# siyi-wind/MDViT

Hardware: AMD Instinct MI355X
Metric: 512x512 images/sec MDViT train step (fwd+bwd, two-sweep, AdamW) (higher is better)
Workload: dtype bf16x3 (fp32 storage; GEMM operands split hi+lo bf16, fp32 accumulate); 1 GPU; MDViT Sup+MLPFM train step, 4 domain(s) x bs=4 per GPU, 512x512, drop_rate=0.1 drop_path=0.1, bf16x3 GEMMs, data-parallel x1

## Files before the change

### include/mdvit_hip.h

```cpp
#ifndef MDVIT_HIP_H
#define MDVIT_HIP_H

#include <stddef.h>
#include <stdint.h>

#ifdef __cplusplus
extern "C" {
#endif

#define MDVIT_ABI_VERSION 1

enum {
    MDVIT_OK = 0,
    MDVIT_E_SHAPE = 1,
    MDVIT_E_DTYPE = 2,
    MDVIT_E_ALIGN = 3,
    MDVIT_E_WORKSPACE = 4,
    MDVIT_E_HIP = 5
};

enum { MDVIT_EPI_NONE = 0, MDVIT_EPI_GELU_DUAL = 1, MDVIT_EPI_DGELU = 2 };
enum { MDVIT_ACT_NONE = 0, MDVIT_ACT_HSWISH = 1, MDVIT_ACT_RELU = 2 };

const char* mdvit_last_error(void);
// ... 274 lines not shown
    float* dW1[MDVIT_DA_MANY_MAX]; float* db1[MDVIT_DA_MANY_MAX]; float* dW2[MDVIT_DA_MANY_MAX]; float* db2[MDVIT_DA_MANY_MAX];
} MdvitDaManyGrads;
size_t mdvit_da_many_ws_bytes(const MdvitDaMany* m, int32_t B);
int mdvit_da_bwd_many(const MdvitDaMany* m, const MdvitDaManyGrads* g, const float* label, float scale, void* ws, size_t ws_bytes, int32_t B, int32_t D, void* stream);
size_t mdvit_da_ws_bytes(int32_t B, int32_t hid, int32_t C);
int mdvit_da_bwd(const float* label, const float* W1, const float* b1, const float* W2, const float* b2, const float* a,
                 const float* e, float scale, float* dW1, float* db1, float* dW2, float* db2, void* ws, size_t ws_bytes,
                 int32_t B, int32_t D, int32_t hid, int32_t C, int32_t heads, void* stream);

size_t mdvit_factoratt_ws_bytes(int32_t B, int32_t N, int32_t C, int32_t heads);
int mdvit_factoratt_fwd(const float* qkv, const float* w3, const float* b3, const float* w5, const float* b5,
                        const float* w7, const float* b7, const float* a, float* out, float* U, float* kmax, float* ksum, float* Mmat,
                        void* ws, size_t ws_bytes, int32_t B, int32_t H, int32_t W, int32_t C, int32_t heads,
                        int32_t s3, int32_t s5, int32_t s7, void* stream);
int mdvit_factoratt_bwd(const float* dout, const float* qkv, const float* out, const float* U,
                        const float* w3, const float* b3, const float* w5, const float* b5, const float* w7, const float* b7,
                        const float* a, const float* kmax, const float* ksum, const float* Mmat,
                        float* dqkv, float* e, float* dw3, float* db3, float* dw5, float* db5, float* dw7, float* db7,
                        void* ws, size_t ws_bytes, int32_t B, int32_t H, int32_t W, int32_t C, int32_t heads,
                        int32_t s3, int32_t s5, int32_t s7, void* stream);
int mdvit_factoratt_wgrad(const float* qkv, void* ws, size_t ws_bytes, float* dw3, float* db3, float* dw5, float* db5,
                          float* dw7, float* db7, int32_t B, int32_t H, int32_t W, int32_t C, int32_t heads,
                          int32_t s3, int32_t s5, int32_t s7, int32_t accumulate, void* stream);

int mdvit_seg_losses_fwd(const float* out, const float* aux, const float* label, double* sums, float* losses, int64_t n, void* stream);
int mdvit_seg_losses_sums(const float* out, const float* aux, const float* label, double* sums, int64_t n, void* stream);
int mdvit_seg_losses_final(const double* sums, float* losses, int64_t n_total, int32_t has_aux, void* stream);
int mdvit_seg_losses_bwd(const float* out, const float* aux, const float* label, const double* sums, const float* g,
                         float* dout, float* daux, int64_t n, float dice_gain, void* stream);
int mdvit_seg_losses_bwd3(const float* out, const float* aux, const float* label, const double* sums, const float* g0, const float* g1, const float* g2,
                          float* dout, float* daux, int64_t n, float dice_gain, void* stream);
int mdvit_seg_losses_groups_sums(const float* out, const float* aux, const float* label, double* sums, int64_t n, int32_t G, void* stream);
int mdvit_seg_losses_groups_final(const double* sums, float* losses, float* per_group, int64_t n_total, int32_t has_aux, int32_t G, void* stream);
int mdvit_seg_losses_groups_bwd(const float* out, const float* aux, const float* label, const double* sums, const float* g0, const float* g1, const float* g2,
                                float* dout, float* daux, int64_t n, int32_t G, float dice_gain, void* stream);

int mdvit_seg_metrics(const float* out, const float* aux, const float* label, uint64_t* counts, float* metrics, int64_t n, void* stream);
size_t mdvit_eval_ws_bytes(int32_t G);
int mdvit_eval_accumulate(const float* out, const float* aux, const float* label, const int32_t* images, const int32_t* domains, int32_t G,
                          int64_t n_per_image, int32_t num_domains, double* acc, int64_t* counts, float* batch_rows, void* ws, size_t ws_bytes, void* stream);
int mdvit_eval_table(const double* acc, int32_t num_domains, float* table, void* stream);
size_t mdvit_eval_images_ws_bytes(int32_t n, int64_t HW);
int mdvit_eval_images(const float* out, const float* aux, const float* label, int32_t n, int64_t HW, int64_t* counts, uint64_t* bits, uint64_t* aux_bits,
                      void* ws, size_t ws_bytes, void* stream);
size_t mdvit_eval_structure_ws_bytes(int32_t n, int32_t H, int32_t W);
int mdvit_eval_structure(const float* pred, const float* label, int32_t n, int32_t H, int32_t W, double* loss, double* sums, void* ws, size_t ws_bytes,
// ... 102 lines not shown
```

### mdvit_amd/_lib.py

```python
from __future__ import annotations

import ctypes as C
import os
import re
from typing import List

_HERE = os.path.dirname(os.path.abspath(__file__))
LIB_PATH = os.environ.get("MDVIT_HIP_LIB") or os.path.join(_HERE, "lib", "libmdvit_hip.so")
HEADER_PATH = os.path.join(_HERE, "..", "include", "mdvit_hip.h")

EPI_NONE, EPI_GELU_DUAL, EPI_DGELU = 0, 1, 2
ACT_NONE, ACT_HSWISH, ACT_RELU = 0, 1, 2

f32p = C.c_void_p
vp = C.c_void_p
i32 = C.c_int32
i64 = C.c_int64
u32 = C.c_uint32
f32 = C.c_float


class GemmDesc(C.Structure):
    _fields_ = [
        ("A", vp), ("B", vp), ("C", vp), ("C2", vp),
# ... 187 lines not shown
    "mdvit_gconv2_3x3_fwd": [vp, vp, vp, vp, i32, i32, i32, i32, vp],
    "mdvit_gconv2_3x3_bwd": [vp, vp, vp, vp, vp, vp, vp, vp, C.c_size_t, i32, i32, i32, i32, i32, vp],
    "mdvit_im2col3x3": [vp, vp, i32, i32, i32, i32, i32, i32, vp],
    "mdvit_col2im3x3": [vp, vp, i32, i32, i32, i32, i32, i32, vp],
    "mdvit_dropout_f32": [vp, vp, i64, f32, u32, u32, vp, vp],
    "mdvit_stemconv_fwd": [vp, vp, vp, i32, i32, i32, i32, i32, vp],
    "mdvit_stemconv_wgrad": [vp, vp, vp, vp, C.c_size_t, i32, i32, i32, i32, i32, i32, vp],
    "mdvit_bn_rowdot_fwd": [vp, vp, vp, vp, vp, vp, vp, vp, i32, i32, i32, f32, u32, u32, vp, i32, vp],
    "mdvit_bn_rowdot_bwd": [vp, vp, vp, vp, vp, vp, vp, vp, vp, vp, vp, vp, vp, C.c_size_t, i32, i32, i32, i32, f32, u32, u32, vp, i32, vp],
    "mdvit_bn_stats": [vp, vp, C.c_size_t, vp, vp, vp, vp, vp, i32, i32, i32, i32, f32, f32, vp],
    "mdvit_bn_eval_prep": [vp, vp, vp, vp, i32, f32, vp],
    "mdvit_bn_apply": [vp, vp, vp, vp, vp, vp, i32, i32, i32, i32, i32, f32, u32, u32, vp, i32, vp],
    "mdvit_bn_bwd": [vp, vp, vp, vp, vp, vp, vp, vp, vp, vp, C.c_size_t, i32, i32, i32, i32, i32, i32, f32, u32, u32, vp, i32, vp],
    "mdvit_upsample_multi_fwd": [vp, vp, vp, i32, vp, vp, i32, i32, i32, i32, vp],
    "mdvit_upsample_multi_bwd": [vp, vp, vp, vp, i32, vp, C.c_size_t, i32, i32, i32, i32, vp],
    "mdvit_upsample_fwd": [vp, vp, vp, i32, i32, i32, i32, i32, i32, vp],
    "mdvit_upsample_bwd": [vp, vp, vp, C.c_size_t, i32, i32, i32, i32, i32, i32, vp],
    "mdvit_upsample_bwd_config": [i32],
    "mdvit_da_fwd": [vp, vp, vp, vp, vp, vp, i32, i32, i32, i32, i32, vp],
    "mdvit_da_bwd": [vp] * 7 + [f32] + [vp] * 4 + [vp, C.c_size_t] + [i32] * 5 + [vp],
    "mdvit_factoratt_fwd": [vp] * 13 + [vp, C.c_size_t] + [i32] * 8 + [vp],
    "mdvit_factoratt_wgrad": [vp, vp, C.c_size_t] + [vp] * 6 + [i32] * 9 + [vp],
    "mdvit_factoratt_bwd": [vp] * 22 + [vp, C.c_size_t] + [i32] * 8 + [vp],
    "mdvit_seg_losses_fwd": [vp, vp, vp, vp, vp, i64, vp],
    "mdvit_adamw_step": [vp, i32, i32, vp, vp, f32, f32, f32, f32, i32, vp],
    "mdvit_adam_step": [vp, i32, i32, vp, vp, f32, f32, f32, f32, i32, i32, vp],
    "mdvit_table_pack": [vp, i32, vp, i32, vp],
    "mdvit_table_unpack": [vp, i32, vp, i32, vp],
    "mdvit_seg_metrics": [vp, vp, vp, vp, vp, i64, vp],
    "mdvit_eval_accumulate": [vp, vp, vp, C.POINTER(i32), C.POINTER(i32), i32, i64, i32, vp, vp, vp, vp, C.c_size_t, vp],
    "mdvit_eval_table": [vp, i32, vp, vp],
    "mdvit_eval_images": [vp, vp, vp, i32, i64, vp, vp, vp, vp, C.c_size_t, vp],
    "mdvit_eval_structure": [vp, vp, i32, i32, i32, vp, vp, vp, C.c_size_t, vp],
    "mdvit_image_normalize_u8": [vp, vp, i32, i32, i32, vp],
    "mdvit_augment_normalize_u8": [vp, vp, vp, vp, vp, vp, i32, i32, i32, vp],
    "mdvit_augment_probe_taps": [f32, f32, i32, i32, C.POINTER(i32), C.POINTER(f32)],
    "mdvit_gather_resize_u8": [vp, vp, vp, vp, i32, vp, i32, vp, vp, i64, i32, i32, i32, i32, i32, vp],
    "mdvit_seg_losses_sums": [vp, vp, vp, vp, i64, vp],
    "mdvit_seg_losses_final": [vp, vp, i64, i32, vp],
    "mdvit_seg_losses_bwd": [vp, vp, vp, vp, vp, vp, vp, i64, f32, vp],
    "mdvit_seg_losses_bwd3": [vp, vp, vp, vp, vp, vp, vp, vp, vp, i64, f32, vp],
    "mdvit_seg_losses_groups_sums": [vp, vp, vp, vp, i64, i32, vp],
    "mdvit_seg_losses_groups_final": [vp, vp, vp, i64, i32, i32, vp],
    "mdvit_seg_losses_groups_bwd": [vp, vp, vp, vp, vp, vp, vp, vp, vp, i64, i32, f32, vp],
    "mdvit_se_adapter_fwd": [C.POINTER(SeAdapterDesc), vp, vp, vp, vp, C.c_size_t, vp],
    "mdvit_se_adapter_bwd": [C.POINTER(SeAdapterDesc)] + [vp] * 10 + [vp, C.c_size_t, vp],
# ... 39 lines not shown
        return _lib
    if not os.path.exists(LIB_PATH):
        raise MdvitHipError(
            f"{LIB_PATH} is missing: build it with `python -m mdvit_amd.build` (hipcc, gfx950). "
            "mdvit_amd has no CPU or PyTorch fallback.")
    lib = C.CDLL(LIB_PATH)
    try:
        _attach_prototypes(lib)
    except AttributeError as e:
        raise MdvitHipError(f"{LIB_PATH} is stale ({e}): rebuild it with `python -m mdvit_amd.build`.") from None
    _lib = lib
    while _on_load:
        _on_load.pop(0)(lib)
    return lib


def _attach_prototypes(lib):
    lib.mdvit_last_error.restype = C.c_char_p
    lib.mdvit_last_error.argtypes = []
    lib.mdvit_version.restype = C.c_int
    lib.mdvit_version.argtypes = []
    lib.mdvit_factoratt_ws_bytes.restype = C.c_size_t
    lib.mdvit_factoratt_ws_bytes.argtypes = [i32, i32, i32, i32]
    lib.mdvit_gemm_ws_bytes.restype = C.c_size_t
    lib.mdvit_gemm_ws_bytes.argtypes = [C.POINTER(GemmDesc)]
    lib.mdvit_gate_bwd_ws_bytes.restype = C.c_size_t
    lib.mdvit_gate_bwd_ws_bytes.argtypes = [i32, i64, i32, i32]
    lib.mdvit_gemm_planes_ws_bytes.restype = C.c_size_t
    lib.mdvit_gemm_planes_ws_bytes.argtypes = [C.POINTER(PlaneGemmDesc)]
    lib.mdvit_bn_rowdot_ws_bytes.restype = C.c_size_t
    lib.mdvit_bn_rowdot_ws_bytes.argtypes = [i32, i32]
    lib.mdvit_bn_ws_bytes.restype = C.c_size_t
    lib.mdvit_bn_ws_bytes.argtypes = [i32, i32, i32]
    lib.mdvit_upsample_multi_bwd_ws_bytes.restype = C.c_size_t
    lib.mdvit_upsample_multi_bwd_ws_bytes.argtypes = [vp, i32, i32, i32, i32]
    lib.mdvit_upsample_bwd_ws_bytes.restype = C.c_size_t
    lib.mdvit_upsample_bwd_ws_bytes.argtypes = [i32] * 6
    lib.mdvit_partials_ws_bytes.restype = C.c_size_t
    lib.mdvit_partials_ws_bytes.argtypes = [i32]
    lib.mdvit_mlp_rc_wgrad_ws_bytes.restype = C.c_size_t
    lib.mdvit_mlp_rc_wgrad_ws_bytes.argtypes = [i32, i32, i32]
    lib.mdvit_block_save_bytes.restype = C.c_size_t
    lib.mdvit_block_save_bytes.argtypes = [C.POINTER(BlockDesc)]
    lib.mdvit_block_fwd_ws_bytes.restype = C.c_size_t
    lib.mdvit_block_fwd_ws_bytes.argtypes = [C.POINTER(BlockDesc)]
    lib.mdvit_block_bwd_ws_bytes.restype = C.c_size_t
# ... 39 lines not shown
```

### mdvit_amd/csrc/attn.hip

```cpp
#include "common.h"
#include "conv_tile.h"

namespace {

constexpr int FA_T = 64;

struct FaGeom {
    int B, H, W, N, C, heads, Ch, s3, s5, s7;
    float scale;
};

typedef float fap_f32x16 __attribute__((ext_vector_type(16)));

template <int CH, bool SOFTMAX>
__global__ __launch_bounds__(256) void fa_partial_kernel(const float* __restrict__ X, long ldx, const float* __restrict__ Y, long ldy,
                                                         const float* __restrict__ ysc, float yscale,
                                                         float* __restrict__ ws_m, float* __restrict__ ws_s, float* __restrict__ ws_P,
                                                         FaGeom g, int NT, int NSUB,
                                                         const float* __restrict__ outp = nullptr, float* __restrict__ dU = nullptr, float* __restrict__ e_part = nullptr) {
    constexpr int GW = CH < 32 ? 32 : CH, NB = (GW + 31) / 32, GQ = GW / 4;
    constexpr int STAGE = 2 * FA_T * GW, RED = 4 * NB * 32 * NB * 32;
    __shared__ __attribute__((aligned(16))) float sm[(STAGE > RED ? STAGE : RED) + 3 * NB * 32 + (SOFTMAX ? 2 * 256 : 0)];
    float* xs = sm;
    float* ys = sm + FA_T * GW;
// ... 1066 lines not shown
}

extern "C" int mdvit_factoratt_wgrad(const float* qkv, void* ws, size_t ws_bytes, float* dw3, float* db3, float* dw5, float* db5,
                                     float* dw7, float* db7, int32_t B, int32_t H, int32_t W, int32_t C, int32_t heads,
                                     int32_t s3, int32_t s5, int32_t s7, int32_t accumulate, void* stream) {
    hipStream_t s = (hipStream_t)stream;
    FaGeom g;
    MDVIT_CHECK_ARG(make_geom(g, B, H, W, C, heads, s3, s5, s7), MDVIT_E_SHAPE, "factoratt_wgrad: bad geometry");
    MDVIT_CHECK_ARG(ws_bytes >= fa_ws_floats(B, g.N, C, heads) * sizeof(float), MDVIT_E_WORKSPACE, "factoratt_wgrad: workspace too small");
    MDVIT_CHECK_ARG(dw3 && db3 && dw5 && db5 && dw7 && db7, MDVIT_E_SHAPE, "factoratt_wgrad: all six outputs are required");
    const int Ch = g.Ch, NT = cdiv(g.N, FA_T);
    const float* dU = (const float*)ws;
    float* wg_part = (float*)ws + 2L * B * g.N * C + (long)B * C * (1 + Ch) + (long)B * NT * C * Ch;
    const int c5 = s3 * Ch, c7 = (s3 + s5) * Ch;
    const CtGeom cg{B, g.H, g.W};
    const int goff[3] = {0, c5, c7}, xoff3[3] = {2 * C, 2 * C + c5, 2 * C + c7}, ncls3[3] = {s3 * Ch, s5 * Ch, s7 * Ch};
    float* const dws[3] = {dw3, dw5, dw7};
    float* const dbs[3] = {db3, db5, db7};
    launch_conv3_wgrad(dU, (long)C, goff, qkv, 3L * C, xoff3, dws, dbs, wg_part, cg, ncls3, s, accumulate);
    MDVIT_LAUNCH_CHECK();
    return MDVIT_OK;
}

extern "C" int mdvit_da_fwd(const float* label, const float* W1, const float* b1, const float* W2, const float* b2, float* a,
                            int32_t B, int32_t D, int32_t hid, int32_t C, int32_t heads, void* stream) {
    MDVIT_CHECK_ARG(B > 0 && D > 0 && hid > 0 && C > 0 && heads > 0 && C % heads == 0, MDVIT_E_SHAPE, "da_fwd: bad shape");
    const int G = max(1, min(1024 / C, hid));
    hipLaunchKernelGGL(da_fwd_kernel, dim3(B), dim3(1024), sizeof(float) * (hid + C + (size_t)(G + 1) * C), (hipStream_t)stream, label, W1, b1, W2, b2, a, D, hid, C, heads);
    MDVIT_LAUNCH_CHECK();
    return MDVIT_OK;
}

extern "C" int mdvit_da_fwd_many(const MdvitDaMany* m, const float* label, int32_t B, int32_t D, void* stream) {
    MDVIT_CHECK_ARG(m && label && B > 0 && D > 0 && m->n > 0 && m->n <= MDVIT_DA_MANY_MAX, MDVIT_E_SHAPE, "da_fwd_many: bad arguments");
    size_t smem = 0;
    for (int i = 0; i < m->n; ++i) {
        const int C = m->C[i], hid = m->hid[i];
        MDVIT_CHECK_ARG(m->W1[i] && m->b1[i] && m->W2[i] && m->b2[i] && m->a[i] && hid > 0 && C > 0 && m->heads[i] > 0 && C % m->heads[i] == 0, MDVIT_E_SHAPE,
                        "da_fwd_many: bad adapter %d", i);
        const int G = max(1, min(1024 / C, hid));
        smem = std::max(smem, sizeof(float) * (hid + C + (size_t)(G + 1) * C));
    }
    MDVIT_CHECK_ARG(smem <= 64 * 1024, MDVIT_E_SHAPE, "da_fwd_many: an adapter needs %zu bytes of LDS", smem);
    hipLaunchKernelGGL(da_fwd_many_kernel, dim3(B, m->n), dim3(1024), smem, (hipStream_t)stream, *m, label, D);
    MDVIT_LAUNCH_CHECK();
    return MDVIT_OK;
// ... 54 lines not shown
```

### mdvit_amd/csrc/conv_tile.h

```cpp
#pragma once
#include "common.h"

namespace {

struct CtGeom { int B, H, W; };

constexpr int CT_TH = 8, CT_TW = 16, CT_CL = 32;

template <int LH, int LW>
struct CtWindow {
    static constexpr int NP = LH * LW, PASSES = (NP + 31) / 32;
    float4 v[PASSES];
    __device__ __forceinline__ void load(const float* __restrict__ x, long ldx, long img, int h0, int w0, int H, int W, int nch) {
        const int q4 = (threadIdx.x & 7) * 4, pl = threadIdx.x >> 3;
#pragma unroll
        for (int i = 0; i < PASSES; ++i) {
            const int p = pl + 32 * i;
            const int hh = h0 + p / LW, ww = w0 + p % LW;
            v[i] = make_float4(0.f, 0.f, 0.f, 0.f);
            if (p < NP && hh >= 0 && hh < H && ww >= 0 && ww < W && q4 < nch)
                v[i] = *reinterpret_cast<const float4*>(x + (img + (long)hh * W + ww) * ldx + q4);
        }
    }
    __device__ __forceinline__ void store(float* __restrict__ sx) const {
        const int q4 = (threadIdx.x & 7) * 4, pl = threadIdx.x >> 3;
#pragma unroll
        for (int i = 0; i < PASSES; ++i) {
            const int p = pl + 32 * i;
            if (p < NP) *reinterpret_cast<float4*>(sx + p * CT_CL + q4) = v[i];
        }
    }
};

template <int LH, int LW>
__device__ __forceinline__ void ct_stage_window(float* __restrict__ sx, const float* __restrict__ x, long ldx, long img,
                                                int h0, int w0, int H, int W, int nch) {
    CtWindow<LH, LW> win;
    win.load(x, ldx, img, h0, w0, H, W, nch);
    win.store(sx);
}

template <int WIN, bool FLIP, int GD = 1, bool PAIR = false>
__device__ __forceinline__ void conv_tile_body(float* __restrict__ sx, float* __restrict__ sw, int cblock,
                                               const float* __restrict__ x, long ldx, int xoff,
                                               const float* __restrict__ w, const float* __restrict__ bias,
                                               float* __restrict__ y, long ldy, int yoff,
                                               int H, int W, int ncls, int tiles_w, int add_center) {
    constexpr int R = WIN / 2, LH = CT_TH + 2 * R, LW = CT_TW + 2 * R;
    const int b = blockIdx.z, c0 = cblock * CT_CL;
    const int th0 = (blockIdx.x / tiles_w) * CT_TH, tw0 = (blockIdx.x % tiles_w) * CT_TW;
    const int cl = threadIdx.x & 31, rl = threadIdx.x >> 5;
    const long img = (long)b * H * W;
    CtWindow<LH, LW> win;
    win.load(x + xoff + c0 / GD, ldx, img, th0 - R, tw0 - R, H, W, (ncls - c0) / GD);
    constexpr int NWQ = (CT_CL * WIN * WIN + 255) / 256;
    float wq[NWQ];
#pragma unroll
    for (int j = 0; j < NWQ; ++j) {
        const int i = threadIdx.x + 256 * j, c = i / (WIN * WIN), t = i % (WIN * WIN);
        const bool ok = i < CT_CL * WIN * WIN && c0 + c < ncls;
        const float wv = w[ok ? (long)(c0 + c) * WIN * WIN + (FLIP ? WIN * WIN - 1 - t : t) : 0];
        wq[j] = ok ? wv : 0.f;
    }
#pragma unroll
    for (int j = 0; j < NWQ; ++j) {
        const int i = threadIdx.x + 256 * j;
        if (i < CT_CL * WIN * WIN) sw[i] = wq[j];
    }
    win.store(sx);
    __syncthreads();
    const int h = th0 + rl;
    if (c0 + cl >= ncls || h >= H) return;
    float acc[CT_TW];
    const float b0 = (!FLIP && bias) ? bias[c0 + cl] : 0.f;
#pragma unroll
    for (int t = 0; t < CT_TW; ++t) acc[t] = b0;
#pragma unroll
    for (int i = 0; i < WIN; ++i) {
        float row[LW], wr[WIN];
#pragma unroll
        for (int t = 0; t < LW; ++t) row[t] = sx[((rl + i) * LW + t) * CT_CL + cl / GD];
        if (i == R && add_center) {
#pragma unroll
            for (int t = 0; t < CT_TW; ++t) acc[t] += row[t + R];
        }
#pragma unroll
        for (int j = 0; j < WIN; ++j) wr[j] = sw[cl * WIN * WIN + i * WIN + j];
#pragma unroll
        for (int t = 0; t < CT_TW; ++t)
#pragma unroll
            for (int j = 0; j < WIN; ++j) acc[t] = fmaf(wr[j], row[t + j], acc[t]);
    }
    if constexpr (PAIR) {
#pragma unroll
        for (int t = 0; t < CT_TW; ++t) {
            const float s2 = acc[t] + __shfl_xor(acc[t], 1);
            if (!(cl & 1) && tw0 + t < W) y[(img + (long)h * W + tw0 + t) * ldy + yoff + (c0 + cl) / 2] = s2;
        }
        return;
    }
// ... 7 lines not shown
                                                           const float* __restrict__ w, const float* __restrict__ bias,
                                                           float* __restrict__ y, long ldy, int yoff,
                                                           int H, int W, int ncls, int tiles_w, int add_center) {
    constexpr int R = WIN / 2, LH = CT_TH + 2 * R, LW = CT_TW + 2 * R;
    __shared__ __attribute__((aligned(16))) float sx[LH * LW * CT_CL];
    __shared__ float sw[CT_CL * WIN * WIN];
    conv_tile_body<WIN, FLIP>(sx, sw, blockIdx.y, x, ldx, xoff, w, bias, y, ldy, yoff, H, W, ncls, tiles_w, add_center);
}

typedef float ct_f2 __attribute__((ext_vector_type(2)));
constexpr int CT2_TH = 16, CT2_TW = 16;

template <int WIN, bool FLIP>
__device__ __forceinline__ void conv_tile2_body(float* __restrict__ sx, float* __restrict__ sw, int cblock,
                                                const float* __restrict__ x, long ldx, int xoff,
                                                const float* __restrict__ w, const float* __restrict__ bias,
                                                float* __restrict__ y, long ldy, int yoff,
                                                int H, int W, int ncls, int tiles_w, int add_center) {
    constexpr int R = WIN / 2, LH = CT2_TH + 2 * R, LW = CT2_TW + 2 * R;
    const int b = blockIdx.z, c0 = cblock * CT_CL;
    const int th0 = (blockIdx.x / tiles_w) * CT2_TH, tw0 = (blockIdx.x % tiles_w) * CT2_TW;
    const int cl = threadIdx.x & 31, rp = threadIdx.x >> 5;
    const long img = (long)b * H * W;
    CtWindow<LH, LW> win;
    win.load(x + xoff + c0, ldx, img, th0 - R, tw0 - R, H, W, ncls - c0);
    constexpr int NWQ = (CT_CL * WIN * WIN + 255) / 256;
    float wq[NWQ];
#pragma unroll
    for (int j = 0; j < NWQ; ++j) {
        const int i = threadIdx.x + 256 * j, c = i / (WIN * WIN), t = i % (WIN * WIN);
        const bool ok = i < CT_CL * WIN * WIN && c0 + c < ncls;
        const float wv = w[ok ? (long)(c0 + c) * WIN * WIN + (FLIP ? WIN * WIN - 1 - t : t) : 0];
        wq[j] = ok ? wv : 0.f;
    }
#pragma unroll
    for (int j = 0; j < NWQ; ++j) {
        const int i = threadIdx.x + 256 * j;
        if (i < CT_CL * WIN * WIN) sw[i] = wq[j];
    }
    win.store(sx);
    __syncthreads();
    const int h = th0 + 2 * rp;
    if (c0 + cl >= ncls || h >= H) return;
    ct_f2 acc[CT2_TW];
    const float b0 = (!FLIP && bias) ? bias[c0 + cl] : 0.f;
#pragma unroll
    for (int t = 0; t < CT2_TW; ++t) acc[t] = ct_f2{b0, b0};
// ... 75 lines not shown
template <bool FLIP>
void launch_conv3(const float* x, long ldx, const int xoff[3], const float* const w[3], const float* const bias[3], float* y, long ldy,
                  const int yoff[3], const CtGeom& g, const int ncls[3], hipStream_t s) {
    Conv3Args a;
    a.x = x; a.ldx = ldx; a.y = y; a.ldy = ldy; a.H = g.H; a.W = g.W; a.tiles_w = cdiv(g.W, CT_TW);
    int total = 0;
    for (int i = 0; i < 3; ++i) {
        a.xoff[i] = xoff[i]; a.yoff[i] = yoff[i]; a.w[i] = w[i]; a.bias[i] = bias ? bias[i] : nullptr; a.ncls[i] = ncls[i];
        a.yb[i] = ncls[i] > 0 ? cdiv(ncls[i], CT_CL) : 0;
        total += a.yb[i];
    }
    if (total == 0) return;
    if (conv_tile_v2() && (long)g.H * g.W >= 4096) {
        a.tiles_w = cdiv(g.W, CT2_TW);
        constexpr int smem = ((CT2_TH + 6) * (CT2_TW + 6) * CT_CL + CT_CL * 49) * 4;
        static bool attr_set = false;
        if (!attr_set) { (void)hipFuncSetAttribute(reinterpret_cast<const void*>(&fa_conv3v2_kernel<FLIP>), hipFuncAttributeMaxDynamicSharedMemorySize, smem); attr_set = true; }
        hipLaunchKernelGGL((fa_conv3v2_kernel<FLIP>), dim3(a.tiles_w * cdiv(g.H, CT2_TH), total, g.B), dim3(256), smem, s, a);
        return;
    }
    hipLaunchKernelGGL((fa_conv3_kernel<FLIP>), dim3(a.tiles_w * cdiv(g.H, CT_TH), total, g.B), dim3(256), 0, s, a);
}

template <int WIN, int GDIV>
__device__ __forceinline__ void conv_tile_wgrad_body(float* __restrict__ sx, float* __restrict__ sg, int bx, int gx, int cb, int b, int nb,
                                                     const float* __restrict__ g, long ldg, int goff,
                                                     const float* __restrict__ x, long ldx, int xoff,
                                                     float* __restrict__ part,
                                                     int H, int W, int ncls, int tiles_w, int tiles_total, int tiles_per_block) {
    constexpr int R = WIN / 2, LH = CT_TH + 2 * R, LW = CT_TW + 2 * R;
    const int c0 = cb * CT_CL;
    const int cl = threadIdx.x & 31, rl8 = threadIdx.x >> 5;
    constexpr int HS = WIN == 3 ? 2 : 1, RPH = CT_TH / HS;
    const int rl = HS == 2 ? (rl8 < 6 ? rl8 % 3 : WIN) : rl8, half = HS == 2 ? rl8 / 3 : 0;
    const long img = (long)b * H * W;
    const bool chan_ok = c0 + cl < ncls;
    float acc[WIN];
    float accb = 0.f;
#pragma unroll
    for (int j = 0; j < WIN; ++j) acc[j] = 0.f;
    const int t_beg = bx * tiles_per_block, t_end = min(tiles_total, t_beg + tiles_per_block);
    for (int tile = t_beg; tile < t_end; ++tile) {
        const int th0 = (tile / tiles_w) * CT_TH, tw0 = (tile % tiles_w) * CT_TW;
        {
            CtWindow<LH, LW> wx;
            CtWindow<CT_TH, CT_TW> wg;
            wx.load(x + xoff + c0, ldx, img, th0 - R, tw0 - R, H, W, ncls - c0);
            wg.load(g + goff + c0 / GDIV, ldg, img, th0, tw0, H, W, (ncls - c0) / GDIV);
            wx.store(sx);
            wg.store(sg);
        }
        __syncthreads();
        if (rl < WIN && chan_ok) {
#pragma unroll 2
            for (int h = half * RPH; h < (half + 1) * RPH; ++h) {
                float row[LW], gr[CT_TW];
#pragma unroll
                for (int t = 0; t < LW; ++t) row[t] = sx[((h + rl) * LW + t) * CT_CL + cl];
#pragma unroll
                for (int t = 0; t < CT_TW; ++t) gr[t] = sg[(h * CT_TW + t) * CT_CL + cl / GDIV];
#pragma unroll
                for (int t = 0; t < CT_TW; ++t) {
                    if (rl == 0) accb += gr[t];
#pragma unroll
                    for (int j = 0; j < WIN; ++j) acc[j] = fmaf(gr[t], row[t + j], acc[j]);
                }
            }
        }
        __syncthreads();
    }
    if (HS == 2) {
        float* s_h = sx;
        if (rl < WIN && half == 1) {
#pragma unroll
            for (int j = 0; j < WIN; ++j) s_h[(rl * (WIN + 1) + j) * CT_CL + cl] = acc[j];
            s_h[(rl * (WIN + 1) + WIN) * CT_CL + cl] = accb;
        }
        __syncthreads();
        if (rl < WIN && half == 0) {
#pragma unroll
            for (int j = 0; j < WIN; ++j) acc[j] += s_h[(rl * (WIN + 1) + j) * CT_CL + cl];
            accb += s_h[(rl * (WIN + 1) + WIN) * CT_CL + cl];
        }
    }
    constexpr int ROW = CT_CL * (WIN * WIN + 1);
    float* prow = part + ((long)cb * nb * gx + (long)b * gx + bx) * ROW + cl * (WIN * WIN + 1);
    if (rl < WIN && half == 0) {
#pragma unroll
        for (int j = 0; j < WIN; ++j) prow[rl * WIN + j] = acc[j];
        if (rl == 0) prow[WIN * WIN] = accb;
    }
}

template <int WIN, int GDIV = 1>
__global__ __launch_bounds__(256) void fa_conv_tile_wgrad_kernel(const float* __restrict__ g, long ldg, int goff,
                                                                 const float* __restrict__ x, long ldx, int xoff,
                                                                 float* __restrict__ part,
                                                                 int H, int W, int ncls, int tiles_w, int tiles_total, int tiles_per_block) {
    constexpr int R = WIN / 2, LH = CT_TH + 2 * R, LW = CT_TW + 2 * R;
    __shared__ __attribute__((aligned(16))) float sx[LH * LW * CT_CL];
    __shared__ __attribute__((aligned(16))) float sg[CT_TH * CT_TW * CT_CL];
    conv_tile_wgrad_body<WIN, GDIV>(sx, sg, blockIdx.x, gridDim.x, blockIdx.y, blockIdx.z, gridDim.z, g, ldg, goff, x, ldx, xoff, part, H, W, ncls, tiles_w, tiles_total,
                                    tiles_per_block);
}

struct Conv3WArgs {
    const float* g; long ldg; int goff[3];
    const float* x; long ldx; int xoff[3];
    float* part[3];
    int H, W, ncls[3], cbs[3], tiles_w, tiles_total, tpb, gx, B;
};
__global__ __launch_bounds__(256) void fa_conv3_wgrad_kernel(Conv3WArgs p) {
    __shared__ __attribute__((aligned(16))) float sx[(CT_TH + 6) * (CT_TW + 6) * CT_CL];
    __shared__ __attribute__((aligned(16))) float sg[CT_TH * CT_TW * CT_CL];
    const unsigned lb = mdvit_xcd_logical_block();
    const int tcb = p.cbs[0] + p.cbs[1] + p.cbs[2];
    int cb = (int)(lb % tcb);
    const unsigned r = lb / tcb;
    const int bx = (int)(r % p.gx), b = (int)(r / p.gx);
    if (cb < p.cbs[0]) { conv_tile_wgrad_body<3, 1>(sx, sg, bx, p.gx, cb, b, p.B, p.g, p.ldg, p.goff[0], p.x, p.ldx, p.xoff[0], p.part[0], p.H, p.W, p.ncls[0], p.tiles_w, p.tiles_total, p.tpb); return; }
    cb -= p.cbs[0];
    if (cb < p.cbs[1]) { conv_tile_wgrad_body<5, 1>(sx, sg, bx, p.gx, cb, b, p.B, p.g, p.ldg, p.goff[1], p.x, p.ldx, p.xoff[1], p.part[1], p.H, p.W, p.ncls[1], p.tiles_w, p.tiles_total, p.tpb); return; }
    cb -= p.cbs[1];
    conv_tile_wgrad_body<7, 1>(sx, sg, bx, p.gx, cb, b, p.B, p.g, p.ldg, p.goff[2], p.x, p.ldx, p.xoff[2], p.part[2], p.H, p.W, p.ncls[2], p.tiles_w, p.tiles_total, p.tpb);
}

template <int WIN, bool FLIP>
void launch_conv_tile(const float* x, long ldx, int xoff, const float* w, const float* bias, float* y, long ldy, int yoff,
                      const CtGeom& g, int ncls, hipStream_t s, int add_center = 0) {
    if (ncls <= 0) return;
    if (WIN > 3 && conv_tile_v2() && (long)g.H * g.W >= 4096) {
        constexpr int R = WIN / 2;
        constexpr int smem = ((CT2_TH + 2 * R) * (CT2_TW + 2 * R) * CT_CL + CT_CL * WIN * WIN) * 4;
        const int tw2 = cdiv(g.W, CT2_TW), th2 = cdiv(g.H, CT2_TH);
        static bool attr_set = false;
        if (!attr_set) { (void)hipFuncSetAttribute(reinterpret_cast<const void*>(&fa_conv_tile2_kernel<WIN, FLIP>), hipFuncAttributeMaxDynamicSharedMemorySize, smem); attr_set = true; }
        hipLaunchKernelGGL((fa_conv_tile2_kernel<WIN, FLIP>), dim3(tw2 * th2, cdiv(ncls, CT_CL), g.B), dim3(256), smem, s,
                           x, ldx, xoff, w, bias, y, ldy, yoff, g.H, g.W, ncls, tw2, add_center);
        return;
    }
    const int tiles_w = cdiv(g.W, CT_TW), tiles_h = cdiv(g.H, CT_TH);
    hipLaunchKernelGGL((fa_conv_tile_kernel<WIN, FLIP>), dim3(tiles_w * tiles_h, cdiv(ncls, CT_CL), g.B), dim3(256), 0, s,
                       x, ldx, xoff, w, bias, y, ldy, yoff, g.H, g.W, ncls, tiles_w, add_center);
}

constexpr int CT_FIN_LANES = 32;
template <int WIN>
// ... 25 lines not shown
        const int c = blockIdx.y * CT_CL + i / T, tap = i % T;
        if (c < ncls) {
            float* dst = tap < WIN * WIN ? dw + (long)c * WIN * WIN + tap : (db ? db + c : nullptr);
            if (dst) *dst = accumulate ? *dst + t : t;
        }
    }
}

void conv_wgrad_plan(const CtGeom& g, int ncls, int& tpb, long& nblk) {
    const int tiles = cdiv(g.W, CT_TW) * cdiv(g.H, CT_TH);
    tpb = 1;
    while (tpb < tiles && (long)cdiv(tiles, tpb * 2) * cdiv(ncls, CT_CL) * g.B >= 512) tpb *= 2;
    nblk = (long)cdiv(tiles, tpb) * cdiv(ncls, CT_CL) * g.B;
}

template <int WIN, int GDIV = 1>
int launch_conv_tile_wgrad(const float* gsrc, long ldg, int goff, const float* x, long ldx, int xoff, float* dw, float* db, float* part,
                           const CtGeom& g, int ncls, hipStream_t s, int accumulate = 0) {
    if (ncls <= 0) return MDVIT_OK;
    const int tiles_w = cdiv(g.W, CT_TW), tiles_h = cdiv(g.H, CT_TH), tiles = tiles_w * tiles_h;
    int tpb; long nblk;
    conv_wgrad_plan(g, ncls, tpb, nblk);
    const int gx = cdiv(tiles, tpb), gy = cdiv(ncls, CT_CL);
    hipLaunchKernelGGL((fa_conv_tile_wgrad_kernel<WIN, GDIV>), dim3(gx, gy, g.B), dim3(256), 0, s,
                       gsrc, ldg, goff, x, ldx, xoff, part, g.H, g.W, ncls, tiles_w, tiles, tpb);
    constexpr int T = WIN * WIN + 1, ROW = CT_CL * T;
    hipLaunchKernelGGL((fa_conv_wgrad_finish_kernel<WIN>), dim3(cdiv(ROW, 32), gy), dim3(32 * CT_FIN_LANES), 0, s, part, gx * g.B, dw, db, ncls, accumulate);
    return MDVIT_OK;
}

inline long conv3_wgrad_rows(const CtGeom& g, const int ncls[3], int& tpb, int& gx) {
    const int tiles = cdiv(g.W, CT_TW) * cdiv(g.H, CT_TH);
    const int tcb = cdiv(ncls[0], CT_CL) + cdiv(ncls[1], CT_CL) + cdiv(ncls[2], CT_CL);
    tpb = 1;
    while (tpb < tiles && (long)cdiv(tiles, tpb * 2) * tcb * g.B >= 512) tpb *= 2;
    gx = cdiv(tiles, tpb);
    return (long)gx * g.B;
}
inline int launch_conv3_wgrad(const float* gsrc, long ldg, const int goff[3], const float* x, long ldx, const int xoff[3], float* const dw[3], float* const db[3],
                              float* part, const CtGeom& g, const int ncls[3], hipStream_t s, int accumulate) {
    int tpb, gx;
    const long rows = conv3_wgrad_rows(g, ncls, tpb, gx);
    Conv3WArgs a;
    a.g = gsrc; a.ldg = ldg; a.x = x; a.ldx = ldx; a.H = g.H; a.W = g.W; a.tiles_w = cdiv(g.W, CT_TW); a.tiles_total = a.tiles_w * cdiv(g.H, CT_TH);
    a.tpb = tpb; a.gx = gx; a.B = g.B;
    const int T[3] = {10, 26, 50};
    float* pp = part;
    int tcb = 0;
    for (int i = 0; i < 3; ++i) {
        a.goff[i] = goff[i]; a.xoff[i] = xoff[i]; a.ncls[i] = ncls[i]; a.cbs[i] = ncls[i] > 0 ? cdiv(ncls[i], CT_CL) : 0;
        a.part[i] = pp;
        pp += (long)a.cbs[i] * rows * CT_CL * T[i];
        tcb += a.cbs[i];
    }
    if (tcb == 0) return MDVIT_OK;
    hipLaunchKernelGGL(fa_conv3_wgrad_kernel, dim3((unsigned)((long)g.B * gx * tcb)), dim3(256), 0, s, a);
    if (a.cbs[0]) hipLaunchKernelGGL((fa_conv_wgrad_finish_kernel<3>), dim3(cdiv(CT_CL * 10, 32), a.cbs[0]), dim3(32 * CT_FIN_LANES), 0, s, a.part[0], (int)rows, dw[0], db[0], ncls[0], accumulate);
    if (a.cbs[1]) hipLaunchKernelGGL((fa_conv_wgrad_finish_kernel<5>), dim3(cdiv(CT_CL * 26, 32), a.cbs[1]), dim3(32 * CT_FIN_LANES), 0, s, a.part[1], (int)rows, dw[1], db[1], ncls[1], accumulate);
    if (a.cbs[2]) hipLaunchKernelGGL((fa_conv_wgrad_finish_kernel<7>), dim3(cdiv(CT_CL * 50, 32), a.cbs[2]), dim3(32 * CT_FIN_LANES), 0, s, a.part[2], (int)rows, dw[2], db[2], ncls[2], accumulate);
    return MDVIT_OK;
}

}
```

Measured before the change: 522.3 images/s.

## Prefetch next tile in conv wgrad loops and add CRPE stencil entry points

The depthwise conv weight-gradient body now software-pipelines its tile loop: when blocks process enough tiles, it loads the next tile's input and gradient windows into registers while computing FMAs on the current shared-memory tile. Window loads use clamped addresses with a validity mask, so the global loads are unconditional. Launch bounds and the forward unroll factor for large windows are also adjusted. New standalone CRPE stencil fwd/bwd C entry points wrap the existing conv3 kernels. The prefetch adds register pressure, which may lower occupancy.

```diff
diff --git a/include/mdvit_hip.h b/include/mdvit_hip.h
--- a/include/mdvit_hip.h
+++ b/include/mdvit_hip.h
@@ -320,6 +320,12 @@
 int mdvit_factoratt_wgrad(const float* qkv, void* ws, size_t ws_bytes, float* dw3, float* db3, float* dw5, float* db5,
                           float* dw7, float* db7, int32_t B, int32_t H, int32_t W, int32_t C, int32_t heads,
                           int32_t s3, int32_t s5, int32_t s7, int32_t accumulate, void* stream);
+int mdvit_crpe_stencil_fwd(const float* qkv, const float* w3, const float* b3, const float* w5, const float* b5, const float* w7, const float* b7,
+                           float* U, int32_t B, int32_t H, int32_t W, int32_t C, int32_t heads, int32_t s3, int32_t s5, int32_t s7, void* stream);
+int mdvit_crpe_stencil_bwd(const float* dU, const float* qkv, const float* w3, const float* w5, const float* w7, float* dV,
+                           float* dw3, float* db3, float* dw5, float* db5, float* dw7, float* db7, void* ws, size_t ws_bytes,
+                           int32_t B, int32_t H, int32_t W, int32_t C, int32_t heads, int32_t s3, int32_t s5, int32_t s7, void* stream);
+size_t mdvit_crpe_stencil_ws_bytes(int32_t B, int32_t H, int32_t W, int32_t C, int32_t heads, int32_t s3, int32_t s5, int32_t s7);
 
 int mdvit_seg_losses_fwd(const float* out, const float* aux, const float* label, double* sums, float* losses, int64_t n, void* stream);
 int mdvit_seg_losses_sums(const float* out, const float* aux, const float* label, double* sums, int64_t n, void* stream);
diff --git a/mdvit_amd/_lib.py b/mdvit_amd/_lib.py
--- a/mdvit_amd/_lib.py
+++ b/mdvit_amd/_lib.py
@@ -233,6 +233,8 @@
     "mdvit_factoratt_fwd": [vp] * 13 + [vp, C.c_size_t] + [i32] * 8 + [vp],
     "mdvit_factoratt_wgrad": [vp, vp, C.c_size_t] + [vp] * 6 + [i32] * 9 + [vp],
     "mdvit_factoratt_bwd": [vp] * 22 + [vp, C.c_size_t] + [i32] * 8 + [vp],
+    "mdvit_crpe_stencil_fwd": [vp] * 8 + [i32] * 8 + [vp],
+    "mdvit_crpe_stencil_bwd": [vp] * 12 + [vp, C.c_size_t] + [i32] * 8 + [vp],
     "mdvit_seg_losses_fwd": [vp, vp, vp, vp, vp, i64, vp],
     "mdvit_adamw_step": [vp, i32, i32, vp, vp, f32, f32, f32, f32, i32, vp],
     "mdvit_adam_step": [vp, i32, i32, vp, vp, f32, f32, f32, f32, i32, i32, vp],
@@ -318,6 +320,8 @@
     lib.mdvit_version.argtypes = []
     lib.mdvit_factoratt_ws_bytes.restype = C.c_size_t
     lib.mdvit_factoratt_ws_bytes.argtypes = [i32, i32, i32, i32]
+    lib.mdvit_crpe_stencil_ws_bytes.restype = C.c_size_t
+    lib.mdvit_crpe_stencil_ws_bytes.argtypes = [i32] * 8
     lib.mdvit_gemm_ws_bytes.restype = C.c_size_t
     lib.mdvit_gemm_ws_bytes.argtypes = [C.POINTER(GemmDesc)]
     lib.mdvit_gate_bwd_ws_bytes.restype = C.c_size_t
diff --git a/mdvit_amd/csrc/attn.hip b/mdvit_amd/csrc/attn.hip
--- a/mdvit_amd/csrc/attn.hip
+++ b/mdvit_amd/csrc/attn.hip
@@ -1112,6 +1112,67 @@
     return MDVIT_OK;
 }
 
+namespace {
+bool crpe_stencil_geom(FaGeom& g, int B, int H, int W, int C, int heads, int s3, int s5, int s7) {
+    return make_geom(g, B, H, W, C, heads, s3, s5, s7) && g.Ch % 4 == 0 && s3 >= 0 && s5 >= 0 && s7 >= 0 && B <= 65535;
+}
+size_t crpe_stencil_ws_floats(const FaGeom& g) {
+    const int ncls[3] = {g.s3 * g.Ch, g.s5 * g.Ch, g.s7 * g.Ch}, T[3] = {10, 26, 50};
+    int tpb, gx;
+    const long rows = conv3_wgrad_rows(CtGeom{g.B, g.H, g.W}, ncls, tpb, gx);
+    size_t n = 0;
+    for (int i = 0; i < 3; ++i) n += (size_t)cdiv(ncls[i], CT_CL) * rows * CT_CL * T[i];
+    return n;
+}
+}
+
+extern "C" size_t mdvit_crpe_stencil_ws_bytes(int32_t B, int32_t H, int32_t W, int32_t C, int32_t heads, int32_t s3, int32_t s5, int32_t s7) {
+    FaGeom g;
+    if (!crpe_stencil_geom(g, B, H, W, C, heads, s3, s5, s7)) return 0;
+    return crpe_stencil_ws_floats(g) * sizeof(float);
+}
+
+extern "C" int mdvit_crpe_stencil_fwd(const float* qkv, const float* w3, const float* b3, const float* w5, const float* b5, const float* w7, const float* b7,
+                                      float* U, int32_t B, int32_t H, int32_t W, int32_t C, int32_t heads, int32_t s3, int32_t s5, int32_t s7, void* stream) {
+    FaGeom g;
+    MDVIT_CHECK_ARG(crpe_stencil_geom(g, B, H, W, C, heads, s3, s5, s7), MDVIT_E_SHAPE, "crpe_stencil_fwd: bad geometry B=%d H=%d W=%d C=%d heads=%d splits=%d/%d/%d", B, H, W, C, heads, s3, s5, s7);
+    MDVIT_CHECK_ARG(qkv && U && w3 && b3 && w5 && b5 && w7 && b7, MDVIT_E_SHAPE, "crpe_stencil_fwd: NULL argument");
+    const int Ch = g.Ch, c5 = s3 * Ch, c7 = (s3 + s5) * Ch;
+    const int xoff[3] = {2 * C, 2 * C + c5, 2 * C + c7}, yoff[3] = {0, c5, c7}, ncls[3] = {s3 * Ch, s5 * Ch, s7 * Ch};
+    const float* const ws3[3] = {w3, w5, w7};
+    const float* const bs3[3] = {b3, b5, b7};
+    launch_conv3<false>(qkv, 3L * C, xoff, ws3, bs3, U, (long)C, yoff, CtGeom{B, g.H, g.W}, ncls, (hipStream_t)stream);
+    MDVIT_LAUNCH_CHECK();
+    return MDVIT_OK;
+}
+
+extern "C" int mdvit_crpe_stencil_bwd(const float* dU, const float* qkv, const float* w3, const float* w5, const float* w7, float* dV,
+                                      float* dw3, float* db3, float* dw5, float* db5, float* dw7, float* db7, void* ws, size_t ws_bytes,
+                                      int32_t B, int32_t H, int32_t W, int32_t C, int32_t heads, int32_t s3, int32_t s5, int32_t s7, void* stream) {
+    hipStream_t s = (hipStream_t)stream;
+    FaGeom g;
+    MDVIT_CHECK_ARG(crpe_stencil_geom(g, B, H, W, C, heads, s3, s5, s7), MDVIT_E_SHAPE, "crpe_stencil_bwd: bad geometry B=%d H=%d W=%d C=%d heads=%d splits=%d/%d/%d", B, H, W, C, heads, s3, s5, s7);
+    const bool want_wgrad = dw3 != nullptr;
+    MDVIT_CHECK_ARG(want_wgrad ? (db3 && dw5 && db5 && dw7 && db7) : !(db3 || dw5 || db5 || dw7 || db7), MDVIT_E_SHAPE,
+                    "crpe_stencil_bwd: the six weight-gradient outputs must be all given or all NULL");
+    MDVIT_CHECK_ARG(dU && (!dV || (w3 && w5 && w7)) && (!want_wgrad || qkv), MDVIT_E_SHAPE, "crpe_stencil_bwd: NULL argument");
+    const int Ch = g.Ch, c5 = s3 * Ch, c7 = (s3 + s5) * Ch;
+    const CtGeom cg{B, g.H, g.W};
+    const int off[3] = {0, c5, c7}, xoff3[3] = {2 * C, 2 * C + c5, 2 * C + c7}, ncls[3] = {s3 * Ch, s5 * Ch, s7 * Ch};
+    if (want_wgrad) {
+        MDVIT_CHECK_ARG(ws && ws_bytes >= crpe_stencil_ws_floats(g) * sizeof(float), MDVIT_E_WORKSPACE, "crpe_stencil_bwd: workspace too small (%zu bytes)", ws_bytes);
+        float* const dws[3] = {dw3, dw5, dw7};
+        float* const dbs[3] = {db3, db5, db7};
+        launch_conv3_wgrad(dU, (long)C, off, qkv, 3L * C, xoff3, dws, dbs, (float*)ws, cg, ncls, s, 0);
+    }
+    if (dV) {
+        const float* const ws3[3] = {w3, w5, w7};
+        launch_conv3<true>(dU, (long)C, off, ws3, nullptr, dV, (long)C, off, cg, ncls, s);
+    }
+    MDVIT_LAUNCH_CHECK();
+    return MDVIT_OK;
+}
+
 extern "C" int mdvit_da_fwd(const float* label, const float* W1, const float* b1, const float* W2, const float* b2, float* a,
                             int32_t B, int32_t D, int32_t hid, int32_t C, int32_t heads, void* stream) {
     MDVIT_CHECK_ARG(B > 0 && D > 0 && hid > 0 && C > 0 && heads > 0 && C % heads == 0, MDVIT_E_SHAPE, "da_fwd: bad shape");
diff --git a/mdvit_amd/csrc/conv_tile.h b/mdvit_amd/csrc/conv_tile.h
--- a/mdvit_amd/csrc/conv_tile.h
+++ b/mdvit_amd/csrc/conv_tile.h
@@ -7,19 +7,29 @@
 
 constexpr int CT_TH = 8, CT_TW = 16, CT_CL = 32;
 
-template <int LH, int LW>
+template <int LH, int LW, bool CLAMP = true>
 struct CtWindow {
     static constexpr int NP = LH * LW, PASSES = (NP + 31) / 32;
     float4 v[PASSES];
+    unsigned ok;
     __device__ __forceinline__ void load(const float* __restrict__ x, long ldx, long img, int h0, int w0, int H, int W, int nch) {
+        static_assert(PASSES <= 32, "one validity bit per pass");
         const int q4 = (threadIdx.x & 7) * 4, pl = threadIdx.x >> 3;
+        const int q4c = q4 < nch ? q4 : 0;
+        ok = 0u;
 #pragma unroll
         for (int i = 0; i < PASSES; ++i) {
             const int p = pl + 32 * i;
             const int hh = h0 + p / LW, ww = w0 + p % LW;
-            v[i] = make_float4(0.f, 0.f, 0.f, 0.f);
-            if (p < NP && hh >= 0 && hh < H && ww >= 0 && ww < W && q4 < nch)
-                v[i] = *reinterpret_cast<const float4*>(x + (img + (long)hh * W + ww) * ldx + q4);
+            if constexpr (!CLAMP) {
+                v[i] = make_float4(0.f, 0.f, 0.f, 0.f);
+                if (p < NP && hh >= 0 && hh < H && ww >= 0 && ww < W && q4 < nch)
+                    v[i] = *reinterpret_cast<const float4*>(x + (img + (long)hh * W + ww) * ldx + q4);
+                continue;
+            }
+            if (p < NP && hh >= 0 && hh < H && ww >= 0 && ww < W && q4 < nch) ok |= 1u << i;
+            const int hc = min(max(hh, 0), H - 1), wc = min(max(ww, 0), W - 1);
+            v[i] = *reinterpret_cast<const float4*>(x + (img + (long)hc * W + wc) * ldx + q4c);
         }
     }
     __device__ __forceinline__ void store(float* __restrict__ sx) const {
@@ -27,7 +37,7 @@
 #pragma unroll
         for (int i = 0; i < PASSES; ++i) {
             const int p = pl + 32 * i;
-            if (p < NP) *reinterpret_cast<float4*>(sx + p * CT_CL + q4) = v[i];
+            if (p < NP) *reinterpret_cast<float4*>(sx + p * CT_CL + q4) = (!CLAMP || (ok >> i & 1u)) ? v[i] : make_float4(0.f, 0.f, 0.f, 0.f);
         }
     }
 };
@@ -51,7 +61,7 @@
     const int th0 = (blockIdx.x / tiles_w) * CT_TH, tw0 = (blockIdx.x % tiles_w) * CT_TW;
     const int cl = threadIdx.x & 31, rl = threadIdx.x >> 5;
     const long img = (long)b * H * W;
-    CtWindow<LH, LW> win;
+    CtWindow<LH, LW, false> win;
     win.load(x + xoff + c0 / GD, ldx, img, th0 - R, tw0 - R, H, W, (ncls - c0) / GD);
     constexpr int NWQ = (CT_CL * WIN * WIN + 255) / 256;
     float wq[NWQ];
@@ -75,7 +85,7 @@
     const float b0 = (!FLIP && bias) ? bias[c0 + cl] : 0.f;
 #pragma unroll
     for (int t = 0; t < CT_TW; ++t) acc[t] = b0;
-#pragma unroll
+#pragma unroll(WIN > 5 ? 2 : WIN)
     for (int i = 0; i < WIN; ++i) {
         float row[LW], wr[WIN];
 #pragma unroll
@@ -129,7 +139,7 @@
     const int th0 = (blockIdx.x / tiles_w) * CT2_TH, tw0 = (blockIdx.x % tiles_w) * CT2_TW;
     const int cl = threadIdx.x & 31, rp = threadIdx.x >> 5;
     const long img = (long)b * H * W;
-    CtWindow<LH, LW> win;
+    CtWindow<LH, LW, false> win;
     win.load(x + xoff + c0, ldx, img, th0 - R, tw0 - R, H, W, ncls - c0);
     constexpr int NWQ = (CT_CL * WIN * WIN + 255) / 256;
     float wq[NWQ];
@@ -251,7 +261,8 @@
     hipLaunchKernelGGL((fa_conv3_kernel<FLIP>), dim3(a.tiles_w * cdiv(g.H, CT_TH), total, g.B), dim3(256), 0, s, a);
 }
 
-template <int WIN, int GDIV>
+constexpr int CT_PF_MIN_TPB = 8, CT_PF3_MIN_TPB = 4;
+template <int WIN, int GDIV, bool PF = true>
 __device__ __forceinline__ void conv_tile_wgrad_body(float* __restrict__ sx, float* __restrict__ sg, int bx, int gx, int cb, int b, int nb,
                                                      const float* __restrict__ g, long ldg, int goff,
                                                      const float* __restrict__ x, long ldx, int xoff,
@@ -269,17 +280,14 @@
 #pragma unroll
     for (int j = 0; j < WIN; ++j) acc[j] = 0.f;
     const int t_beg = bx * tiles_per_block, t_end = min(tiles_total, t_beg + tiles_per_block);
-    for (int tile = t_beg; tile < t_end; ++tile) {
+    CtWindow<LH, LW> wx;
+    CtWindow<CT_TH, CT_TW> wg;
+    auto request = [&](int tile) {
         const int th0 = (tile / tiles_w) * CT_TH, tw0 = (tile % tiles_w) * CT_TW;
-        {
-            CtWindow<LH, LW> wx;
-            CtWindow<CT_TH, CT_TW> wg;
-            wx.load(x + xoff + c0, ldx, img, th0 - R, tw0 - R, H, W, ncls - c0);
-            wg.load(g + goff + c0 / GDIV, ldg, img, th0, tw0, H, W, (ncls - c0) / GDIV);
-            wx.store(sx);
-            wg.store(sg);
-        }
-        __syncthreads();
+        wx.load(x + xoff + c0, ldx, img, th0 - R, tw0 - R, H, W, ncls - c0);
+        wg.load(g + goff + c0 / GDIV, ldg, img, th0, tw0, H, W, (ncls - c0) / GDIV);
+    };
+    auto fmas = [&]() {
         if (rl < WIN && chan_ok) {
 #pragma unroll 2
             for (int h = half * RPH; h < (half + 1) * RPH; ++h) {
@@ -296,9 +304,23 @@
                 }
             }
         }
+    };
+    request(t_beg);
+    wx.store(sx);
+    wg.store(sg);
+    __syncthreads();
+    for (int tile = t_beg; tile + 1 < t_end; ++tile) {
+        if constexpr (PF) request(tile + 1);
+        fmas();
         __syncthreads();
-    }
+        if constexpr (!PF) request(tile + 1);
+        wx.store(sx);
+        wg.store(sg);
+        __syncthreads();
+    }
+    fmas();
     if (HS == 2) {
+        __syncthreads();
         float* s_h = sx;
         if (rl < WIN && half == 1) {
 #pragma unroll
@@ -321,15 +343,15 @@
     }
 }
 
-template <int WIN, int GDIV = 1>
-__global__ __launch_bounds__(256) void fa_conv_tile_wgrad_kernel(const float* __restrict__ g, long ldg, int goff,
+template <int WIN, int GDIV = 1, bool PF = true>
+__global__ __launch_bounds__(256, WIN == 3 ? 4 : 2) void fa_conv_tile_wgrad_kernel(const float* __restrict__ g, long ldg, int goff,
                                                                  const float* __restrict__ x, long ldx, int xoff,
                                                                  float* __restrict__ part,
                                                                  int H, int W, int ncls, int tiles_w, int tiles_total, int tiles_per_block) {
     constexpr int R = WIN / 2, LH = CT_TH + 2 * R, LW = CT_TW + 2 * R;
     __shared__ __attribute__((aligned(16))) float sx[LH * LW * CT_CL];
     __shared__ __attribute__((aligned(16))) float sg[CT_TH * CT_TW * CT_CL];
-    conv_tile_wgrad_body<WIN, GDIV>(sx, sg, blockIdx.x, gridDim.x, blockIdx.y, blockIdx.z, gridDim.z, g, ldg, goff, x, ldx, xoff, part, H, W, ncls, tiles_w, tiles_total,
+    conv_tile_wgrad_body<WIN, GDIV, PF>(sx, sg, blockIdx.x, gridDim.x, blockIdx.y, blockIdx.z, gridDim.z, g, ldg, goff, x, ldx, xoff, part, H, W, ncls, tiles_w, tiles_total,
                                     tiles_per_block);
 }
 
@@ -339,6 +361,7 @@
     float* part[3];
     int H, W, ncls[3], cbs[3], tiles_w, tiles_total, tpb, gx, B;
 };
+template <bool PF>
 __global__ __launch_bounds__(256) void fa_conv3_wgrad_kernel(Conv3WArgs p) {
     __shared__ __attribute__((aligned(16))) float sx[(CT_TH + 6) * (CT_TW + 6) * CT_CL];
     __shared__ __attribute__((aligned(16))) float sg[CT_TH * CT_TW * CT_CL];
@@ -347,11 +370,11 @@
     int cb = (int)(lb % tcb);
     const unsigned r = lb / tcb;
     const int bx = (int)(r % p.gx), b = (int)(r / p.gx);
-    if (cb < p.cbs[0]) { conv_tile_wgrad_body<3, 1>(sx, sg, bx, p.gx, cb, b, p.B, p.g, p.ldg, p.goff[0], p.x, p.ldx, p.xoff[0], p.part[0], p.H, p.W, p.ncls[0], p.tiles_w, p.tiles_total, p.tpb); return; }
+    if (cb < p.cbs[0]) { conv_tile_wgrad_body<3, 1, PF>(sx, sg, bx, p.gx, cb, b, p.B, p.g, p.ldg, p.goff[0], p.x, p.ldx, p.xoff[0], p.part[0], p.H, p.W, p.ncls[0], p.tiles_w, p.tiles_total, p.tpb); return; }
     cb -= p.cbs[0];
-    if (cb < p.cbs[1]) { conv_tile_wgrad_body<5, 1>(sx, sg, bx, p.gx, cb, b, p.B, p.g, p.ldg, p.goff[1], p.x, p.ldx, p.xoff[1], p.part[1], p.H, p.W, p.ncls[1], p.tiles_w, p.tiles_total, p.tpb); return; }
+    if (cb < p.cbs[1]) { conv_tile_wgrad_body<5, 1, PF>(sx, sg, bx, p.gx, cb, b, p.B, p.g, p.ldg, p.goff[1], p.x, p.ldx, p.xoff[1], p.part[1], p.H, p.W, p.ncls[1], p.tiles_w, p.tiles_total, p.tpb); return; }
     cb -= p.cbs[1];
-    conv_tile_wgrad_body<7, 1>(sx, sg, bx, p.gx, cb, b, p.B, p.g, p.ldg, p.goff[2], p.x, p.ldx, p.xoff[2], p.part[2], p.H, p.W, p.ncls[2], p.tiles_w, p.tiles_total, p.tpb);
+    conv_tile_wgrad_body<7, 1, PF>(sx, sg, bx, p.gx, cb, b, p.B, p.g, p.ldg, p.goff[2], p.x, p.ldx, p.xoff[2], p.part[2], p.H, p.W, p.ncls[2], p.tiles_w, p.tiles_total, p.tpb);
 }
 
 template <int WIN, bool FLIP>
@@ -423,8 +446,12 @@
     int tpb; long nblk;
     conv_wgrad_plan(g, ncls, tpb, nblk);
     const int gx = cdiv(tiles, tpb), gy = cdiv(ncls, CT_CL);
-    hipLaunchKernelGGL((fa_conv_tile_wgrad_kernel<WIN, GDIV>), dim3(gx, gy, g.B), dim3(256), 0, s,
-                       gsrc, ldg, goff, x, ldx, xoff, part, g.H, g.W, ncls, tiles_w, tiles, tpb);
+    if (tpb >= CT_PF_MIN_TPB)
+        hipLaunchKernelGGL((fa_conv_tile_wgrad_kernel<WIN, GDIV, true>), dim3(gx, gy, g.B), dim3(256), 0, s,
+                           gsrc, ldg, goff, x, ldx, xoff, part, g.H, g.W, ncls, tiles_w, tiles, tpb);
+    else
+        hipLaunchKernelGGL((fa_conv_tile_wgrad_kernel<WIN, GDIV, false>), dim3(gx, gy, g.B), dim3(256), 0, s,
+                           gsrc, ldg, goff, x, ldx, xoff, part, g.H, g.W, ncls, tiles_w, tiles, tpb);
     constexpr int T = WIN * WIN + 1, ROW = CT_CL * T;
     hipLaunchKernelGGL((fa_conv_wgrad_finish_kernel<WIN>), dim3(cdiv(ROW, 32), gy), dim3(32 * CT_FIN_LANES), 0, s, part, gx * g.B, dw, db, ncls, accumulate);
     return MDVIT_OK;
@@ -455,7 +482,8 @@
         tcb += a.cbs[i];
     }
     if (tcb == 0) return MDVIT_OK;
-    hipLaunchKernelGGL(fa_conv3_wgrad_kernel, dim3((unsigned)((long)g.B * gx * tcb)), dim3(256), 0, s, a);
+    if (tpb >= CT_PF3_MIN_TPB) hipLaunchKernelGGL(fa_conv3_wgrad_kernel<true>, dim3((unsigned)((long)g.B * gx * tcb)), dim3(256), 0, s, a);
+    else hipLaunchKernelGGL(fa_conv3_wgrad_kernel<false>, dim3((unsigned)((long)g.B * gx * tcb)), dim3(256), 0, s, a);
     if (a.cbs[0]) hipLaunchKernelGGL((fa_conv_wgrad_finish_kernel<3>), dim3(cdiv(CT_CL * 10, 32), a.cbs[0]), dim3(32 * CT_FIN_LANES), 0, s, a.part[0], (int)rows, dw[0], db[0], ncls[0], accumulate);
     if (a.cbs[1]) hipLaunchKernelGGL((fa_conv_wgrad_finish_kernel<5>), dim3(cdiv(CT_CL * 26, 32), a.cbs[1]), dim3(32 * CT_FIN_LANES), 0, s, a.part[1], (int)rows, dw[1], db[1], ncls[1], accumulate);
     if (a.cbs[2]) hipLaunchKernelGGL((fa_conv_wgrad_finish_kernel<7>), dim3(cdiv(CT_CL * 50, 32), a.cbs[2]), dim3(32 * CT_FIN_LANES), 0, s, a.part[2], (int)rows, dw[2], db[2], ncls[2], accumulate);
```

After: 522.9 images/s (median of 3 runs). About the same (+0.1%).
